# thomasantony/splat

Hardware: AMD Instinct MI355X
Metric: frames_per_sec (higher is better)
Workload: dtype f32

## Files before the change

### splat_amd/csrc/splat_api.hip

```cpp
#include <algorithm>
#include <cmath>
#include <cstdio>
#include <cstdlib>
#include <cstring>
#include <mutex>
#include <new>
#include <string>
#include <unordered_map>
#include <vector>

#include "splat_context.h"

using namespace splat;

static thread_local std::string g_create_error;
static std::mutex g_ledger_mu;
static std::unordered_map<void*, std::pair<splat_ctx*, size_t>> g_ledger;

namespace splat {
CommState** ctx_comm_slot(splat_ctx* c) { return &c->comm; }
hipStream_t ctx_stream(splat_ctx* c) { return c->stream; }
hipStream_t frame_stream(splat_ctx* c) { return (c->last_lane && c->comp2) ? c->comp2 : c->stream; }
int frame_tail(splat_ctx* c) {
    if (c->last_ring < 0 || !c->ring[c->last_ring].used) return SPLAT_OK;
// ... 491 lines not shown
        HIP_TRY(c, hipEventRecord(s.ev_ready, f.ss));
        HIP_TRY(c, hipStreamWaitEvent(cs, s.ev_ready, 0));
    }
    if (retained) launch_status_set(cs, f.d_st, c->ret_set.status);
    HIP_TRY(c, f.mark(5, cs));
    uint2* iters = nullptr;
    c->iters_valid = false;
    if (want_iters) {
        if (c->iters_alloc < m * 4u) {
            dfree(c->d_iters); c->iters_alloc = 0;
            HIP_TRY(c, dmalloc(c, &c->d_iters, sizeof(uint2) * (size_t)m * 4u));
            c->iters_alloc = m * 4u;
        }
        HIP_TRY(c, hipMemsetAsync(c->d_iters, 0, sizeof(uint2) * (size_t)m * 4u, cs));
        iters = c->d_iters;
        c->iters_valid = true;
    }
    CompositeArgs comp{};
    comp.s = cs; comp.knobs = &c->knobs; comp.n_tiles = m; comp.fc = c->fc; comp.recs = s.recs; comp.argb = d_argb; comp.status = f.d_st; comp.orig = c->orig;
    comp.fused_sort_max = retained ? 0u : c->fused_sort_max; comp.iters = iters; comp.keep_keys = want_iters || f.retain == SPLAT_RETAIN_WRITER;
    comp.pair_walk = pd.pair_walk != 0;
    comp.libm_exp = (c->cfg.mode & SPLAT_MODE_LIBM_EXP) != 0; comp.clear_first = c->clear_first;
    comp.lists = f.lists; comp.lists.near_m = pd.near_cap ? s.near_m : nullptr;
    comp.keys = f.keys; comp.keys.keys2 = pd.comp_sorts != 0 ? s.keys2 : nullptr;
    if (retained) {
        const bool near = c->ret_set.near_cap != 0u;
        comp.lists.near_m = near ? s.near_m : nullptr; comp.keys.keys2 = near ? s.keys2 : nullptr;
    }
    comp.hints = hint_table(c);
    if (c->knobs.dbg_stage_cache != 0u && f.retain == SPLAT_RETAIN_WRITER) {
        const size_t waves = (size_t)c->m_alloc * 4u;
        if (!c->stage_nv || !c->stage_mask) {
            dfree(c->stage_nv); dfree(c->stage_mask);
            HIP_TRY(c, dmalloc(c, &c->stage_nv, sizeof(unsigned int) * waves));
            HIP_TRY(c, dmalloc(c, &c->stage_mask, sizeof(unsigned long long) * 32u * waves));
        }
        HIP_TRY(c, hipMemsetAsync(c->stage_nv, 0, sizeof(unsigned int) * waves, cs));
        c->ret_set.frames = 0;
    }
    if (retained && c->knobs.dbg_stage_cache != 0u && c->stage_nv && c->stage_mask) {
        comp.stage_nv = c->stage_nv; comp.stage_mask = c->stage_mask;
        if (c->knobs.dbg_stage_cache == 2u && c->ret_set.frames >= 2u)
            HIP_TRY(c, hipMemsetAsync(c->stage_mask, 0, sizeof(unsigned long long) * 32u * (size_t)c->m_alloc * 4u, cs));
        c->ret_set.frames++;
    }
    comp.refine = c->fc.close_width == 0.0f ? pd.refine : 0u;
    launch_composite(comp);
    c->last_near = retained ? c->ret_set.near_cap != 0u : pd.near_cap != 0u;
    HIP_TRY(c, f.mark(6, cs));
    if (want_iters) HIP_TRY(c, hipMemcpyAsync(&c->h_status[f.r], f.d_st, sizeof(FrameStatus), hipMemcpyDeviceToHost, cs));
    HIP_TRY(c, hipEventRecord(f.ev->e[7], cs));
    return SPLAT_OK;
}

int decide_retention(splat_ctx* c, const splat_camera* cam, int* action) {
    splat_retain_input in;
    std::memset(&in, 0, sizeof in);
    static_assert(sizeof(splat_camera) + 2 * sizeof(int32_t) <= sizeof in.cam, "the camera and the slab fit the decision's words");
    std::memcpy(in.cam, cam, sizeof(splat_camera));
    const int32_t slab[2] = {c->slab0, c->slab1};
    std::memcpy(reinterpret_cast<unsigned char*>(in.cam) + sizeof(splat_camera), slab, sizeof slab);
    in.epoch = c->bin_epoch; in.still_frames = c->pol.still_frames;
    in.enabled = (c->retain_lists != 0 && c->knobs.dbg_ntiles == 0u) ? 1 : 0;
    in.overlap = c->overlap; in.one_pass = c->fc.bucket_cap ? 1 : 0;
    splat_retain_decision d;
    const int wr = c->ret_set.ring;
    for (int pass = 0; pass < 2; ++pass) {
        if (c->ret.writer == 1u && wr >= 0) {
            const volatile FrameStatus* hs = &c->h_status[wr];
            in.writer_arrived = hs->arrived; in.writer_overflow = hs->overflow; in.writer_redone = hs->redone;
        }
        if (splat_retain_decide(&c->ret, &in, &d) != 0) return fail(c, SPLAT_ERR_INVALID, "retention refused its input");
        if (pass == 0 && d.wait_for_writer != 0 && wr >= 0 && c->ring[wr].used) {
            HIP_TRY(c, hipEventSynchronize(c->ring[wr].e[7]));
// ... 411 lines not shown
    if (const char* e5 = std::getenv("SPLAT_BUCKETS")) { c->use_buckets = std::atoi(e5) != 0; c->env_pinned |= 1u << SPLAT_OPT_ONE_PASS_BINNING; }
    if (const char* e7 = std::getenv("SPLAT_CULL")) { c->cull_blocks = std::atoi(e7) != 0; c->env_pinned |= 1u << SPLAT_OPT_BLOCK_CULLING; }
    if (const char* e8 = std::getenv("SPLAT_DBG_TIGHT_GRIDS")) c->tight_grids = std::atoi(e8) != 0;
    option_from_env(c, SPLAT_OPT_PAIR_WALK, "SPLAT_PAIR_BLEND", -1, 1);
    if (const char* e6 = std::getenv("SPLAT_BUCKET_BYTES")) { c->bucket_bytes = std::strtoull(e6, nullptr, 10); c->env_pinned |= 1u << SPLAT_OPT_KEY_BUFFER_BYTES; }
    option_from_env(c, SPLAT_OPT_REGION_SPARE, "SPLAT_REGION_SPARE", 1, 1e9);
    if (const char* er = std::getenv("SPLAT_OVERFLOW_REDO")) { c->overflow_redo = std::min(2, std::max(0, std::atoi(er))); c->env_pinned |= 1u << SPLAT_OPT_OVERFLOW_REDO; }
    if (const char* en = std::getenv("SPLAT_NEAR_KEYS")) {
        const int v = std::atoi(en);
        c->near_cap = v <= 0 ? 0u : (unsigned int)std::min(2048, std::max(64, v));
        c->env_pinned |= 1u << SPLAT_OPT_NEAR_SELECT_KEYS;
    }
    option_from_env(c, SPLAT_OPT_HOST_ZERO_COPY, "SPLAT_HOST_ZERO_COPY", 0, 1);
    option_from_env(c, SPLAT_OPT_COUNT_FIRST, "SPLAT_COUNT_FIRST", 0, 2);
    if (const char* kg = std::getenv("SPLAT_KEYS_PER_GAUSSIAN")) {
        const int v = std::atoi(kg);
        c->keys_per_gaussian = v <= 0 ? 0u : (unsigned int)std::min(256, std::max(4, v));
        c->env_pinned |= 1u << SPLAT_OPT_KEYS_PER_GAUSSIAN;
    }
    option_from_env(c, SPLAT_OPT_LARGE_SPLAT_TILES, "SPLAT_LARGE_TILES", -1, 1048576);
    option_from_env(c, SPLAT_OPT_LARGE_LIST_MIN, "SPLAT_LARGE_LIST_MIN", -1, 1e9);
    option_from_env(c, SPLAT_OPT_START_REFINE, "SPLAT_START_REFINE", 0, 1);
    option_from_env(c, SPLAT_OPT_RETAIN_LISTS, "SPLAT_RETAIN", 0, 1);
    if (const char* lm = std::getenv("SPLAT_LAYOUT_MOTION")) c->layout_motion = std::atoi(lm) != 0 ? 1 : 0;
    if (const char* k1 = std::getenv("SPLAT_SORT_RADIX_MIN")) c->knobs.sort_radix_min = (unsigned int)std::max(0, std::atoi(k1));
    if (const char* k2 = std::getenv("SPLAT_SCAN_THREADS")) c->knobs.scan_threads = std::atoi(k2);
    if (const char* k3 = std::getenv("SPLAT_DBG_NTILES")) c->knobs.dbg_ntiles = (unsigned int)std::max(0, std::atoi(k3));
    if (const char* k8 = std::getenv("SPLAT_DBG_SELECT_STRIDE")) c->knobs.dbg_select_stride = (unsigned int)std::max(0, std::atoi(k8));
    if (const char* k10 = std::getenv("SPLAT_START_HINTS")) { c->start_hints = std::min(2, std::max(0, std::atoi(k10))); c->env_pinned |= 1u << SPLAT_OPT_START_HINTS; }
    if (const char* k7 = std::getenv("SPLAT_DBG_ONE_PASS_SELECT")) c->one_pass_select = std::atoi(k7) != 0;
    if (const char* k11 = std::getenv("SPLAT_DBG_KEYS2_ENTRIES")) c->knobs.dbg_keys2_entries = std::strtoull(k11, nullptr, 10);
    if (const char* k9 = std::getenv("SPLAT_DBG_HINT_RADIUS")) c->knobs.dbg_hint_radius = std::atoi(k9);
    if (const char* k12 = std::getenv("SPLAT_DBG_SELECT_BLIND")) c->knobs.dbg_select_blind = std::atoi(k12) != 0 ? 1u : 0u;
    if (const char* k13 = std::getenv("SPLAT_DBG_STAGE_CACHE")) c->knobs.dbg_stage_cache = (unsigned int)std::min(2, std::max(0, std::atoi(k13)));
    if (const char* k5 = std::getenv("SPLAT_DBG_STARTS")) c->knobs.dbg_starts = std::atoi(k5) != 0 ? 1u : 0u;
    if (const char* k4 = std::getenv("SPLAT_COMP_LDS_PAD")) c->knobs.comp_lds_pad = (unsigned int)std::max(0, std::atoi(k4));
    if (const char* k1p = std::getenv("SPLAT_K1_LDS_PAD")) c->knobs.k1_lds_pad = (unsigned int)std::min(48 * 1024, std::max(0, std::atoi(k1p)));
    auto bail = [&](const char* what, hipError_t err) {
        g_create_error = std::string(what) + ": " + hipGetErrorString(err);
        splat_destroy(c);
        return SPLAT_ERR_HIP;
    };
    if ((e = hipSetDevice(cfg->device)) != hipSuccess) return bail("hipSetDevice", e);
    if ((e = init_device_kernels()) != hipSuccess) return bail("hipFuncSetAttribute", e);
    if ((e = hipStreamCreateWithFlags(&c->stream, hipStreamNonBlocking)) != hipSuccess) return bail("hipStreamCreate", e);
    c->own_stream = true;
    {
        int lo = 0, hi = 0;
        (void)hipDeviceGetStreamPriorityRange(&lo, &hi);
        int prio = c->pipeline >= 6 ? (lo + hi) / 2 : hi;
        if (const char* ep = std::getenv("SPLAT_BIN_PRIO")) prio = std::atoi(ep) > 0 ? hi : (std::atoi(ep) < 0 ? lo : (lo + hi) / 2);
        if ((e = hipStreamCreateWithPriority(&c->bin_stream, hipStreamNonBlocking, prio)) != hipSuccess) return bail("hipStreamCreate", e);
        if ((e = hipStreamCreateWithPriority(&c->sort_stream, hipStreamNonBlocking, prio)) != hipSuccess) return bail("hipStreamCreate", e);
    }
    if (c->overlap >= 2 && c->pipeline) { if ((e = ensure_copy_stream(c)) != hipSuccess) return bail("hipStreamCreate", e); c->comp2 = c->copy_stream; }
    for (Slot& s : c->slots) {
        if ((e = dmalloc(c, &s.d_status, sizeof(FrameStatus))) != hipSuccess) return bail("hipMalloc(status)", e);
        if ((e = fill_now(s.d_status, 0, sizeof(FrameStatus))) != hipSuccess) return bail("fill_now(status)", e);
        if ((e = hipEventCreateWithFlags(&s.ev_ready, hipEventDisableTiming)) != hipSuccess) return bail("hipEventCreate", e);
        if ((e = hipEventCreateWithFlags(&s.ev_binned, hipEventDisableTiming)) != hipSuccess) return bail("hipEventCreate", e);
    }
    if ((e = dmalloc(c, &c->d_status_ring, sizeof(FrameStatus) * EV_RING)) != hipSuccess) return bail("hipMalloc(status ring)", e);
    if ((e = fill_now(c->d_status_ring, 0, sizeof(FrameStatus) * EV_RING)) != hipSuccess) return bail("fill_now(status ring)", e);
    if ((e = hipHostMalloc(&c->h_status, sizeof(FrameStatus) * EV_RING, hipHostMallocCoherent)) != hipSuccess) return bail("hipHostMalloc(status)", e);
    std::memset(c->h_status, 0, sizeof(FrameStatus) * EV_RING);
    for (auto& s : c->ring)
// ... 489 lines not shown
    if (n != c->n) return fail(c, SPLAT_ERR_INVALID, "record count mismatch");
    if (n == 0) return SPLAT_OK;
    int rc = splat_sync(c);
    if (rc != SPLAT_OK) return rc;
    if (c->last_slot < 0) return fail(c, SPLAT_ERR_INVALID, "no frame rendered yet");
    rc = ensure_two_pass_buffers(c, c->slots[c->last_slot]);
    if (rc != SPLAT_OK) return rc;
    const Slot& s = c->slots[c->last_slot];
    std::vector<Rec> r(n); std::vector<float> d(n); std::vector<ushort4> q(n);
    HIP_TRY(c, hipMemcpy(r.data(), s.recs, sizeof(Rec) * n, hipMemcpyDeviceToHost));
    {
        bump_epoch(c);
        FrameConst fc = c->fc;
        fc.bucket_cap = 0; fc.cull_blocks = 0;
        Slot& sl = c->slots[c->last_slot];
        HIP_TRY(c, hipMemsetAsync(sl.counts, 0, sizeof(unsigned int) * ((size_t)c->n_tiles + 1), c->stream));
        sl.layout_valid = false; sl.flip = 0;
        HIP_TRY(c, hipMemsetAsync(s.d_status, 0, sizeof(FrameStatus), c->stream));
        BinArgs k1{};
        k1.s = c->stream; k1.knobs = &c->knobs; k1.scene = {c->n, c->planes, c->orig, nullptr}; k1.fc = fc; k1.recs = s.recs; k1.depth = s.depth; k1.rect = s.rect;
        k1.vislist = s.vislist; k1.bin.cursors = s.counts; k1.status = s.d_status;
        launch_preprocess(k1);
        HIP_TRY(c, hipMemsetAsync(s.counts, 0, sizeof(unsigned int) * ((size_t)c->n_tiles + 1), c->stream));
        HIP_TRY(c, hipMemsetAsync(s.d_status, 0, sizeof(FrameStatus), c->stream));
        HIP_TRY(c, hipStreamSynchronize(c->stream));
    }
    HIP_TRY(c, hipMemcpy(d.data(), s.depth, sizeof(float) * n, hipMemcpyDeviceToHost));
    HIP_TRY(c, hipMemcpy(q.data(), s.rect, sizeof(ushort4) * n, hipMemcpyDeviceToHost));
    rc = ensure_h_orig(c);
    if (rc != SPLAT_OK) return rc;
    for (uint64_t j = 0; j < n; ++j) {
        const uint64_t i = c->h_orig[j];
        splat_record& o = out[i];
        o.cx = r[j].a.x; o.cy = r[j].a.y; o.hx = r[j].a.z; o.hy = r[j].a.w;
        o.conic_a = r[j].b.x; o.conic_b = c->fc.y_up ? r[j].b.y : -r[j].b.y; o.conic_c = r[j].b.z; o.opacity = r[j].b.w;
        o.r = r[j].c.x; o.g = r[j].c.y; o.b = r[j].c.z; o.depth = d[j];
        o.px0 = q[j].x; o.px1 = q[j].y; o.py0 = q[j].z; o.py1 = q[j].w;
    }
    return SPLAT_OK;
}

#if SPLAT_K1X == 30 || SPLAT_K1X == 31
int splat_debug_k1_stamps(splat_ctx* c, unsigned long long* out, unsigned long long n_words) {
    if (!c || c->last_slot < 0) return SPLAT_ERR_INVALID;
    (void)sync_all(c);
    return hipMemcpy(out, c->slots[c->last_slot].depth, n_words * 8, hipMemcpyDeviceToHost) == hipSuccess ? SPLAT_OK : SPLAT_ERR_HIP;
}
int splat_debug_k1_hwid(splat_ctx* c, unsigned long long* out, unsigned long long n_words) {
    if (!c || c->last_slot < 0) return SPLAT_ERR_INVALID;
    (void)sync_all(c);
    return hipMemcpy(out, c->slots[c->last_slot].rect, n_words * 8, hipMemcpyDeviceToHost) == hipSuccess ? SPLAT_OK : SPLAT_ERR_HIP;
}
#endif

int splat_debug_near_state(splat_ctx* c, unsigned int* lens, unsigned int* near_m, unsigned int* need_hint, unsigned int m) {
    if (!c || c->last_slot < 0 || m != c->n_tiles) return SPLAT_ERR_INVALID;
    (void)sync_all(c);
    const Slot& s = c->slots[c->last_slot];
    bool ok = hipMemcpy(lens, s.lens, sizeof(unsigned int) * m, hipMemcpyDeviceToHost) == hipSuccess;
    ok = ok && hipMemcpy(near_m, s.near_m, sizeof(unsigned int) * m, hipMemcpyDeviceToHost) == hipSuccess;
    ok = ok && hipMemcpy(need_hint, hint_table(c).needs(), sizeof(unsigned int) * HintTable::NEED_PLANES * m, hipMemcpyDeviceToHost) == hipSuccess;
    return ok ? SPLAT_OK : SPLAT_ERR_HIP;
}

int splat_debug_probe_failures(splat_ctx* c, uint64_t* n) {
    if (!c || !n || c->last_slot < 0) return SPLAT_ERR_INVALID;
// ... 57 lines not shown
```

### splat_amd/csrc/splat_context.h

```cpp
#ifndef SPLAT_CONTEXT_H
#define SPLAT_CONTEXT_H
#include <string>
#include <vector>

#include "splat_internal.h"
#include "../../include/splat_policy.h"
#include "../../include/splat_retain.h"

#define HIP_TRY(ctx, expr)                                                                             \
    do {                                                                                               \
        hipError_t _e = (expr);                                                                        \
        if (_e != hipSuccess) {                                                                        \
            (ctx)->err = std::string(#expr) + ": " + hipGetErrorString(_e);                            \
            return SPLAT_ERR_HIP;                                                                      \
        }                                                                                              \
    } while (0)

namespace splat {
constexpr int N_EV = 9;
constexpr int N_TIMES = 6;
constexpr int EV_RING = 32;
static_assert(EV_RING == SPLAT_POLICY_RING, "the frame policy sees the whole status ring");
constexpr int N_SLOTS = 4;

// ... 82 lines not shown
    unsigned int* upd_bad = nullptr;
    unsigned char* upd_dirty = nullptr;
    float ply_ms[3] = {0.0f, 0.0f, 0.0f};
    float upload_sort_ms = 0.0f;
    splat::Slot slots[splat::N_SLOTS];
    unsigned int m_alloc = 0;
    uint64_t cap = 0;
    uint64_t cap2 = 0;
    uint64_t keys2_want = 0;
    bool use_buckets = true;
    bool bucket_failed = false;
    uint64_t bucket_bytes = 128ull << 30;
    uint64_t layout_want = 0;
    unsigned int layout_m = 0;
    bool last_one_pass = false;
    unsigned int* zero_layout = nullptr;
    uint64_t dev_bytes = 0, dev_bytes_peak = 0;
    splat::LaunchKnobs knobs;
    float region_spare = 4.0f;
    uint64_t frame_idx = 0;
    uint64_t bin_idx = 0;
    int retain_lists = 1;
    uint64_t bin_epoch = 0;
    splat_retain_state ret{};
    uint64_t frames_retained = 0;
    struct RetainSet {
        int slot = -1, ring = -1;
        unsigned int near_cap = 0;
        splat::FrameStatus status{};
        unsigned int frames = 0;
    } ret_set;
    unsigned int* stage_nv = nullptr;
    unsigned long long* stage_mask = nullptr;
    int last_slot = -1;
    bool last_lists_in_memory = false;
    splat::FrameStatus* h_status = nullptr;
    splat::FrameStatus* d_status_ring = nullptr;
    bool clear_first = false;
    uint32_t* d_img = nullptr;
    size_t img_cap = 0;
    static constexpr int S_IMGS = 4;
    uint32_t* s_img[S_IMGS] = {};
    size_t s_cap = 0;
    hipStream_t copy_stream = nullptr;
    hipEvent_t s_rendered[S_IMGS] = {}, s_copied[S_IMGS] = {};
    const uint32_t* s_dst[S_IMGS] = {};
    bool s_used[S_IMGS] = {};
    uint64_t s_idx = 0;
    int s_ring[S_IMGS] = {-1, -1, -1, -1};
    splat_camera s_cam[S_IMGS] = {};
    int slab0 = 0, slab1 = -1;
    splat::EvSet ring[splat::EV_RING];
    int ring_next = 0;
    int last_ring = -1;
    double acc_ms[splat::N_TIMES] = {0, 0, 0, 0, 0, 0};
    uint64_t acc_frames = 0;
    splat::FrameConst fc{};
    unsigned int n_tiles = 0;
    uint64_t overflow_want = 0;
    bool bucket_overflow = false;
    bool sort_hint = false, sort_grid_miss = false;
    unsigned int hint_ge8192 = 0, hint_ge2048 = 0, hint_ge16384 = 0;
    int pair_mode = -1;
    uint64_t hint_pairs = 0; unsigned int hint_maxlen = 0; unsigned int hint_large = 0, hint_window = 0;
    unsigned int grid_big = 0, grid_mid = 0, grid_long = 0;
    splat::FrameStatus last{};
// ... 48 lines not shown
```

### splat_amd/csrc/splat_internal.h

```cpp
#ifndef SPLAT_INTERNAL_H
#define SPLAT_INTERNAL_H
#include <hip/hip_runtime.h>
#include <stdint.h>

#include "../../include/splat_hip.h"

#ifndef SPLAT_K1X
#define SPLAT_K1X 0
#endif
#ifndef SPLAT_EXP_STAGE2
#define SPLAT_EXP_STAGE2 0
#endif
#ifndef SPLAT_EXP_K1DUMMY
#define SPLAT_EXP_K1DUMMY 0
#endif
#ifndef SPLAT_EXP_SKIPFULL
#define SPLAT_EXP_SKIPFULL 0
#endif
#ifndef SPLAT_EXP_SORT2
#define SPLAT_EXP_SORT2 0
#endif
#ifndef SPLAT_EXP_K1DROP
#define SPLAT_EXP_K1DROP 0
#endif

namespace splat {

constexpr int TILE = SPLAT_TILE;
constexpr int SCENE_PLANES = 16;
constexpr int LIVE_PLANES = 10;


struct FrameConst {
    float view[16];
    float proj[16];
    float w, h;
    float htanx, htany, focal;
    float cam[3];
    float lowpass;
    int sh_dim;
    int y_up, sample_half, zclip;
    float zmin, zmax;
    int W, H;
    int tiles_x;
// ... 26 lines not shown
    unsigned long long n_sort_fallback;
    unsigned int n_near_tiles;
    unsigned int n_near_fallback;
    unsigned int n_large;
    unsigned int n_window;
    unsigned int n_ge8192, n_ge2048;
    unsigned int n_ge16384;
    unsigned int redone;
    unsigned int n_long_keys;
    unsigned int arrived;
    unsigned int n_probe_fail;
    unsigned int pad_;
    unsigned long long n_blocks_culled;
    unsigned long long layout_total;
};

struct Rec {
    float4 a;
    float4 b;
    float4 c;
};

struct LaunchKnobs {
    unsigned int sort_radix_min = 128;
    int scan_threads = 0;
    unsigned int dbg_ntiles = 0;
    unsigned int comp_lds_pad = 0;
    unsigned int k1_lds_pad = 0;
    unsigned int dbg_select_stride = 0;
    unsigned long long dbg_keys2_entries = 0;
    int dbg_hint_radius = -1;
    unsigned int dbg_select_blind = 0;
    unsigned int dbg_starts = 0;
    unsigned int dbg_stage_cache = 1;
};

struct HintTable {
    unsigned int* base;
    size_t stride;

    static constexpr unsigned int NEED_PLANE = 0u, NEED_PLANES = 4u;
    static constexpr unsigned int DEPTH_PLANE = NEED_PLANE + NEED_PLANES, DEPTH_PLANES = 1u;
    static constexpr unsigned int START_PLANE = DEPTH_PLANE + DEPTH_PLANES, START_PLANES = 4u;
    static constexpr unsigned int REFINE_PLANE = START_PLANE + START_PLANES, REFINE_PLANES = 4u;
    static constexpr unsigned int HINT_WORDS = 13u;
    static_assert(DEPTH_PLANE == 4u && START_PLANE == 5u && REFINE_PLANE == 9u && REFINE_PLANE + REFINE_PLANES == HINT_WORDS,
                  "the four parts tile the table exactly");

    unsigned int* plane(unsigned int k) const { return base ? base + k * stride : nullptr; }
    unsigned int* needs() const { return plane(NEED_PLANE); }
    unsigned int* select_depth() const { return plane(DEPTH_PLANE); }
    unsigned int* starts() const { return plane(START_PLANE); }
    unsigned int* refinement() const { return plane(REFINE_PLANE); }
    size_t words() const { return HINT_WORDS * stride; }
    size_t bytes() const { return sizeof(unsigned int) * words(); }
};

void launch_pack_scene(hipStream_t s, uint64_t n, const float* pos4, const float* cov3d, const float* opacity,
                       const float* sh, const unsigned int* perm, float4* planes);
void launch_cov3d(hipStream_t s, uint64_t n, const float* scales3, const float* rot4, float* cov3d);
size_t scene_order_small_bytes(uint64_t n);
void launch_scene_order(hipStream_t s, uint64_t n, const float* pos4, uint32_t* pingpong, void* small, unsigned int* orig,
                        hipEvent_t sort_begin = nullptr, hipEvent_t sort_end = nullptr);
void launch_block_bounds(hipStream_t s, uint64_t n, const float* pos4, const float* cov3d, const unsigned int* orig, BlockBounds* bounds);

void launch_ply_decode(hipStream_t s, const splat_ply_layout& lay, const void* d_rows, float* pos4, float* scales3,
// ... 106 lines not shown
struct SortArgs {
    hipStream_t s; const LaunchKnobs* knobs; unsigned int n_tiles; SortGrids grids; TileLists lists; KeyBuffers keys; FrameStatus* status;
    const unsigned int* orig;
    unsigned int fused_sort_max;
};
void launch_sort(const SortArgs& a);

struct SelectArgs {
    hipStream_t s; const LaunchKnobs* knobs; unsigned int n_tiles; TileLists lists; KeyBuffers keys; FrameStatus* status;
    const unsigned int* orig;
    unsigned int near_cap;
    const unsigned int* need_hint;
    unsigned int* near_thr;
    unsigned int tiles_x, tile_rows;
    unsigned int grid;
    bool at_rest;
    int hint_radius;
};
void launch_select(const SelectArgs& a);

struct CompositeArgs {
    hipStream_t s; const LaunchKnobs* knobs; unsigned int n_tiles; FrameConst fc;
    TileLists lists;
    KeyBuffers keys;
    const Rec* recs; uint32_t* argb; FrameStatus* status; const unsigned int* orig;
    unsigned int fused_sort_max;
    uint2* iters;
    bool keep_keys;
    bool pair_walk;
    bool libm_exp;
    bool clear_first;
    HintTable hints;
    unsigned int refine;
    unsigned int* stage_nv;
    unsigned long long* stage_mask;
};
void launch_composite(const CompositeArgs& a);
void launch_status_set(hipStream_t s, FrameStatus* status, const FrameStatus& v);
hipError_t init_device_kernels();

struct CommState;
CommState** ctx_comm_slot(splat_ctx* c);
hipStream_t ctx_stream(splat_ctx* c);
hipStream_t frame_stream(splat_ctx* c);
int ctx_device(const splat_ctx* c);
int frame_tail(splat_ctx* c);
int ctx_quiesce(splat_ctx* c);
int ctx_fail(splat_ctx* c, int code, const char* msg);
void comm_release(CommState* s);

}
#endif
```

### splat_amd/csrc/splat_kernels.hip

```cpp
#include <algorithm>
#include <cstddef>
#include <cstdlib>
#include <type_traits>

#include "splat_internal.h"
#include "splat_device_math.h"

namespace splat {
static constexpr unsigned long long KERNELS_EXP2F_TAB[32] = {
    0x3ff0000000000000ull, 0x3fefd9b0d3158574ull, 0x3fefb5586cf9890full, 0x3fef9301d0125b51ull, 0x3fef72b83c7d517bull,
    0x3fef54873168b9aaull, 0x3fef387a6e756238ull, 0x3fef1e9df51fdee1ull, 0x3fef06fe0a31b715ull, 0x3feef1a7373aa9cbull,
    0x3feedea64c123422ull, 0x3feece086061892dull, 0x3feebfdad5362a27ull, 0x3feeb42b569d4f82ull, 0x3feeab07dd485429ull,
    0x3feea47eb03a5585ull, 0x3feea09e667f3bcdull, 0x3fee9f75e8ec5f74ull, 0x3feea11473eb0187ull, 0x3feea589994cce13ull,
    0x3feeace5422aa0dbull, 0x3feeb737b0cdc5e5ull, 0x3feec49182a3f090ull, 0x3feed503b23e255dull, 0x3feee89f995ad3adull,
    0x3feeff76f2fb5e47ull, 0x3fef199bdd85529cull, 0x3fef3720dcef9069ull, 0x3fef5818dcfba487ull, 0x3fef7c97337b9b5full,
    0x3fefa4afa2a490daull, 0x3fefd0765b6e4540ull};
constexpr bool exp2f_tab_is_the_headers() {
    for (int i = 0; i < 32; ++i) if (KERNELS_EXP2F_TAB[i] != EXP2F_TAB_HOST[i]) return false;
    return true;
}
static_assert(exp2f_tab_is_the_headers(), "splat_kernels.hip's copy of EXP2F_TAB differs from splat_device_math.h's");
}


// ... 2245 lines not shown
    unsigned long long* h = keys2 + off2[tile];
    merge(g, r1, g + r1, r2 - r1, h);
    merge(g + r2, r3 - r2, g + r3, n - r3, h + r2);
    __syncthreads();
    merge(h, r2, h + r2, n - r2, g);
}

__device__ __forceinline__ unsigned long long uniform_u64(unsigned long long v) {
    return ((unsigned long long)(unsigned int)__builtin_amdgcn_readfirstlane((int)(v >> 32)) << 32) |
           (unsigned long long)(unsigned int)__builtin_amdgcn_readfirstlane((int)(unsigned int)v);
}

struct WaveLds { float4 a[64]; float4 b[64]; float4 c[64]; };

#ifndef SPLAT_REFINE_MIN_STEP
#define SPLAT_REFINE_MIN_STEP 8
#endif
#ifndef SPLAT_COMP_WAVES
#define SPLAT_COMP_WAVES 1
#endif
struct CompArgs {
    FrameConst fc;
    const unsigned int* offsets; const unsigned int* order; const unsigned int* lens;
    unsigned long long* keys; const Rec* recs; uint32_t* argb; FrameStatus* status;
    unsigned int fused_sort_max, radix_min;
    uint2* iters;
    unsigned int keep_keys, clear_first;
    const unsigned int* orig;
    unsigned long long* keys2; const unsigned int* near_m;
    unsigned int* need_hint; unsigned int* start_hint; const unsigned int* off2;
    unsigned int* probe_hint;
    unsigned int refine;
    unsigned int* stage_nv; unsigned long long* stage_mask;
};
typedef const __attribute__((address_space(4))) CompArgs* KernArgs;
template <bool PAIR, bool LIBM, bool KEEP>
static __device__ void repair_tile(KernArgs ka, unsigned int smem_lds, unsigned int exptab_lds, unsigned int item, bool again);

template <bool PAIR, bool LIBM, int LONGM, bool KEEP = false>
__device__ __forceinline__ void composite_tile(unsigned char* smem, const unsigned long long* exptab, const unsigned int item, const FrameConst& fc,
                                               const unsigned int* __restrict__ offsets, const unsigned int* __restrict__ order,
                                               const unsigned int* __restrict__ lens, unsigned long long* __restrict__ keys,
                                               const Rec* __restrict__ recs, uint32_t* __restrict__ argb,
                                               FrameStatus* __restrict__ status, unsigned int fused_sort_max,
                                               unsigned int radix_min, uint2* __restrict__ iters, unsigned int keep_keys,
                                               const unsigned int* __restrict__ orig, const unsigned int clear_first,
                                               unsigned long long* __restrict__ keys2, const unsigned int* __restrict__ near_m,
                                               unsigned int* __restrict__ need_hint, unsigned int* __restrict__ start_hint,
                                               const unsigned int* __restrict__ off2, KernArgs ka ,
                                               const bool walk_this_wave = true, const bool second_walk = false ) {
    auto late = [&]() -> KernArgs {
        unsigned long long p = (unsigned long long)(size_t)ka;
        asm volatile("" : "+s"(p));
        return (KernArgs)(size_t)p;
    };
    static_assert(sizeof(WaveLds) * 4 <= sort_lds_bytes<256, 2048>(), "staging fits the sort workspace");
    WaveLds* slds = reinterpret_cast<WaveLds*>(smem);
    const unsigned int tile = (unsigned int)__builtin_amdgcn_readfirstlane((int)order[item]);
    const unsigned int tid = threadIdx.x;
    const unsigned int beg = __builtin_amdgcn_readfirstlane(offsets[tile]);
    const unsigned int end = beg + __builtin_amdgcn_readfirstlane(lens[tile]);
    if (beg == end) {
        if (clear_first) {
            const KernArgs k = late();
            const int tiles_x = k->fc.tiles_x, W = k->fc.W, H = k->fc.H, r0 = k->fc.row_px0, r1 = k->fc.row_px1;
            const int txx0 = (int)(tile % (unsigned int)tiles_x), tyy0 = (int)(tile / (unsigned int)tiles_x) + k->fc.tile_row0;
// ... 279 lines not shown
                B2 = blend_channel(B2, ia, ab);
            }
        };
        blend_one(alpha0, (f2){q4.x, q4.y}, q5.x);
        blend_one(alpha1, (f2){q4.z, q4.w}, q5.z);
    };
    auto run = [&](auto BRt, unsigned int start) -> unsigned int {
        constexpr bool BR = decltype(BRt)::value;
        Rec r;
        unsigned int kb = start < end ? (end - 1u - start) >> 6 : 0u;
        unsigned int bsN = start, cntN = start < end ? (end - (kb << 6)) - start : 0u;
        if (cntN) fetch(bsN, cntN, r);
        while (cntN) {
            const unsigned int bs = bsN, cnt = cntN;
            const bool reuse = kb < nA;
            const unsigned int abase = (end - lb >= ((kb + 1u) << 6)) ? end - ((kb + 1u) << 6) : lb;
            const bool keep = KEEP && keeping && !reuse && kb < 32u && bs == abase;
            const unsigned int k = stage(r, cnt, bs, true, false, PAIR, reuse ? (int)kb : -1, bs - abase, keep ? (int)kb : -1);
            bsN = bs + cnt; cntN = min(64u, end - bsN); kb -= cntN ? 1u : 0u;
            if (cntN) fetch(bsN, cntN, r);
            if constexpr (PAIR) {
                const float4* P4 = reinterpret_cast<const float4*>(&L);
                for (unsigned int j = 0; j < (k + 1u) / 2u; ++j)
                    shade_pair(BRt, P4[6 * j], P4[6 * j + 1], P4[6 * j + 2], P4[6 * j + 3], P4[6 * j + 4], P4[6 * j + 5]);
            } else {
                for (unsigned int j = 0; j < k; ++j) shade(BRt, L.a[j], L.b[j], L.c[j]);
            }
            itB += k;
            if (BR && __builtin_amdgcn_ballot_w64(inside & ((R2 - R > cw) | (G2 - G > cw) | (B2 - B > cw))) == 0ull) return bsN;
        }
        return end;
    };
    unsigned int start = ws;
    while (!need_far) {
        if (start <= lb) {
            if (has_far) { need_far = true; break; }
            R = (float)((old >> 16) & 0xffu); G = (float)((old >> 8) & 0xffu); B = (float)(old & 0xffu);
            run(std::false_type{}, lb);
            break;
        }
        R = G = B = 0.0f; R2 = G2 = B2 = 255.0f;
        const unsigned int pos = run(std::true_type{}, start);
        const bool open = __builtin_amdgcn_ballot_w64(inside & ((R2 - R > cw) | (G2 - G > cw) | (B2 - B > cw))) != 0ull;
        if (!open) {
            R = truncf((R + R2) * 0.5f); G = truncf((G + G2) * 0.5f); B = truncf((B + B2) * 0.5f);
            if (pos < end) run(std::false_type{}, pos);
            break;
        }
        if (probe != 0u && !(probe >> 31)) {
            probe |= 0x80000000u;
            const KernArgs kr = late();
            const unsigned int g = (unsigned int)__builtin_amdgcn_readfirstlane((int)kr->start_hint[tile * 4u + wave]);
            if (lane == 0) atomicAdd(&kr->status->n_probe_fail, 1u);
            if (g > end - start && g < end - lb) { start = end - g; continue; }
        }
        if (lane == 0) atomicAdd(&late()->status->n_fallback, 1ull);
        const unsigned int depth = end - start;
        start = (start - lb > depth) ? start - depth : lb;
    }
    const float A = (alast < 0.0f) ? (float)(old >> 24) : truncf(alast * 255.0f);
    const KernArgs kl = late();
    uint2* const iters_l = kl->iters;
    if (iters_l != nullptr && lane == 0) {
        const unsigned int kk = kl->keep_keys;
        uint2 v = (kk & 2u) ? make_uint2(end - beg, end - max(start, beg)) : make_uint2(itA, itB);
        if (second_walk && !(kk & 2u)) { const uint2 o = iters_l[item * 4u + wave]; v.x += o.x; v.y += o.y; }
        iters_l[item * 4u + wave] = v;
    }
    if constexpr (LONGM != 0) {
        unsigned int* const need_l = kl->need_hint;
        if (need_l != nullptr && end - beg > 2048u && lane == 0u) need_l[tile * 4u + wave] = need_far ? 0xffffffffu : end - max(start, lb);
    }
    unsigned int* const start_l = kl->start_hint;
    if (start_l != nullptr && early && !need_far && (scanned || start != ws) && lane == 0u) {
        unsigned int used = max(end - max(start, lb), 1u);
        if (!has_far && used > (end - beg) - ((end - beg) >> 2)) used = end - beg;
        start_l[tile * 4u + wave] = used;
    }
    if (probe != 0u && lane == 0u) {
        const bool failed = (probe >> 31) != 0u;
        const unsigned int half = (probe & 0xffffu) >> 1;
        const unsigned int step = failed ? (half >= (unsigned int)SPLAT_REFINE_MIN_STEP ? half : 0u) : probe;
        if (!failed) start_l[tile * 4u + wave] = end - ws;
        kl->probe_hint[tile * 4u + wave] = (kl->refine & 0xffff0000u) | step;
    }
    if (KEEP && keeping && !need_far && max(start, lb) < end) {
        const unsigned int s = max(start, lb), kf = (end - 1u - s) >> 6;
        const unsigned int ab = (end - lb >= ((kf + 1u) << 6)) ? end - ((kf + 1u) << 6) : lb;
        const unsigned int nv_new = min(kf + (s == ab ? 1u : 0u), 32u);
        unsigned int* const nv_l = kl->stage_nv;
        const unsigned int nv_old = (unsigned int)__builtin_amdgcn_readfirstlane((int)nv_l[tile * 4u + wave]);
        if (nv_new > nv_old) {
            __builtin_amdgcn_fence(__ATOMIC_RELEASE, "wavefront");
            __builtin_amdgcn_wave_barrier();
            if (lane >= nv_old && lane < nv_new) kl->stage_mask[(size_t)(tile * 4u + wave) * 32u + lane] = wmask[lane];
            if (lane == 0u) nv_l[tile * 4u + wave] = nv_new;
            __builtin_amdgcn_fence(__ATOMIC_ACQUIRE, "wavefront");
            __builtin_amdgcn_wave_barrier();
        }
    }
    if (need_far) return true;
    if (inside)
        kl->argb[(size_t)py * kl->fc.W + px] = ((uint32_t)A << 24) | ((uint32_t)R << 16) | ((uint32_t)G << 8) | (uint32_t)B;
    return false;
    };
    if constexpr (LONGM != 2) {
        (void)walk_list();
    } else {
        const bool again = walk_list();
        if (has_far && __syncthreads_or(again ? 1 : 0) != 0) {
            if (tid == 0u) atomicAdd(&late()->status->n_near_fallback, 1u);
            repair_tile<PAIR, LIBM, KEEP>(ka, (unsigned int)(size_t)(__attribute__((address_space(3))) unsigned char*)smem,
                                    (unsigned int)(size_t)(__attribute__((address_space(3))) const unsigned long long*)exptab, item, again);
        }
    }
}

template <bool PAIR, bool LIBM, bool KEEP>
static __device__ __attribute__((noinline)) void repair_tile(KernArgs ka, unsigned int smem_lds, unsigned int exptab_lds, unsigned int item, bool again) {
    const unsigned long long kp = uniform_u64((unsigned long long)(size_t)ka);
    const KernArgs k = (KernArgs)(size_t)kp;
    unsigned char* const smem = (unsigned char*)(__attribute__((address_space(3))) unsigned char*)(size_t)__builtin_amdgcn_readfirstlane((int)smem_lds);
    const unsigned long long* const exptab = (const unsigned long long*)(__attribute__((address_space(3))) const unsigned long long*)(size_t)__builtin_amdgcn_readfirstlane((int)exptab_lds);
    const unsigned int it = (unsigned int)__builtin_amdgcn_readfirstlane((int)item);
    FrameConst fc;
    {
        const __attribute__((address_space(4))) unsigned int* src = (const __attribute__((address_space(4))) unsigned int*)&k->fc;
        unsigned int* dst = reinterpret_cast<unsigned int*>(&fc);
#pragma unroll
        for (unsigned int q = 0; q < sizeof(FrameConst) / 4u; ++q) dst[q] = src[q];
    }
    composite_tile<PAIR, LIBM, 1>(smem, exptab, it, fc, k->offsets, k->order, k->lens, k->keys, k->recs, k->argb, k->status, k->fused_sort_max, k->radix_min,
                                  k->iters, k->keep_keys, k->orig, k->clear_first, k->keys2, nullptr, k->need_hint, k->start_hint, k->off2, k, again, true);
    if (threadIdx.x == 0u) {
        const unsigned int tile = k->order[it];
        const_cast<unsigned int*>(k->near_m)[tile] = k->lens[tile];
        unsigned int* const nv_l = KEEP ? k->stage_nv : nullptr;
        if (nv_l != nullptr) { nv_l[tile * 4u + 0u] = 0u; nv_l[tile * 4u + 1u] = 0u; nv_l[tile * 4u + 2u] = 0u; nv_l[tile * 4u + 3u] = 0u; }
    }
}

__global__ __launch_bounds__(256) void select_near_kernel(const unsigned int* __restrict__ offsets, const unsigned int* __restrict__ order,
                                                          const unsigned int* __restrict__ lens, unsigned long long* __restrict__ keys,
                                                          unsigned long long* __restrict__ keys2, FrameStatus* __restrict__ status,
                                                          const unsigned int* __restrict__ orig, unsigned int radix_min, unsigned int near_cap,
                                                          const unsigned int* __restrict__ need_hint, unsigned int* __restrict__ near_m,
                                                          unsigned int tiles_x, unsigned int tile_rows, unsigned int* __restrict__ near_thr,
                                                          unsigned int n_slots, unsigned int at_rest, const unsigned int* __restrict__ off2,
                                                          int hint_radius, unsigned int blind) {
    __shared__ __attribute__((aligned(16))) unsigned char smem[sort_lds_bytes<256, 2048>()];
    if (status->overflow) return;
  for (unsigned int slot = blockIdx.x; slot < n_slots; slot += gridDim.x) {
    const unsigned int tile = (unsigned int)__builtin_amdgcn_readfirstlane((int)order[slot]);
    const unsigned int n = (unsigned int)__builtin_amdgcn_readfirstlane((int)lens[tile]);
    if (n < 2048u) return;
    if (n == 2048u) continue;
    const unsigned int beg = (unsigned int)__builtin_amdgcn_readfirstlane((int)offsets[tile]);
    unsigned long long* const k2 = keys2 + (unsigned int)__builtin_amdgcn_readfirstlane((int)off2[tile]);
    unsigned int want = near_cap, deepest, thr = 0u;
    {
        unsigned int* const word = reinterpret_cast<unsigned int*>(smem);
        if (threadIdx.x < 64u) {
            const uint4 h4 = reinterpret_cast<const uint4*>(need_hint)[tile];
            unsigned int d0 = max(max(h4.x, h4.y), max(h4.z, h4.w));
            if (hint_radius > 0) {
                const int D = 2 * hint_radius + 1;
                unsigned int nb = 0u;
                for (int idx = (int)threadIdx.x; idx < D * D; idx += 64) {
                    const int tx = (int)(tile % tiles_x) + idx % D - hint_radius, ty = (int)(tile / tiles_x) + idx / D - hint_radius;
                    if (tx >= 0 && ty >= 0 && tx < (int)tiles_x && ty < (int)tile_rows) {
                        const uint4 q = reinterpret_cast<const uint4*>(need_hint)[(unsigned int)ty * tiles_x + (unsigned int)tx];
// ... 231 lines not shown
                               status, orig, off2);
    }
    if (grid_mid)
    hipLaunchKernelGGL((sort_tiles_kernel<512, 8192>), dim3(grid_mid), dim3(512), (sort_lds_bytes<512, 8192>()), s, offsets, order,
                       lens, keys, keys2, status, 2048u, radix_min, 0, 0u, 1u, orig, off2);
    if (fused_sort_max < 2048u)
        hipLaunchKernelGGL((sort_tiles_kernel<256, 2048>), dim3(n_tiles), dim3(256), (sort_lds_bytes<256, 2048>()), s, offsets, order,
                           lens, keys, keys2, status, fused_sort_max, radix_min, 0, 0u, 1u, orig, off2);
}
void launch_select(const SelectArgs& a) {
    const unsigned int n_tiles = a.n_tiles;
    if (!n_tiles) return;
    const unsigned int* off2 = a.lists.off2;
    if (!off2) off2 = a.lists.offsets;
    int hint_radius = a.hint_radius;
    unsigned int grid = a.grid;
    if (a.knobs->dbg_hint_radius >= 0) hint_radius = a.knobs->dbg_hint_radius;
    if (a.knobs->dbg_select_stride) grid = (n_tiles + a.knobs->dbg_select_stride - 1u) / a.knobs->dbg_select_stride;
    if (!grid) grid = (n_tiles + 7u) / 8u;
    hipLaunchKernelGGL(select_near_kernel, dim3(std::min(grid, n_tiles)), dim3(256), 0, a.s, a.lists.offsets, a.lists.order, a.lists.lens, a.keys.keys, a.keys.keys2, a.status, a.orig, a.knobs->sort_radix_min,
                       std::min(std::max(a.near_cap, 64u), 2048u), a.need_hint, a.lists.near_m, a.tiles_x, a.tile_rows, a.near_thr, n_tiles, a.at_rest ? 1u : 0u, off2, std::min(std::max(hint_radius, 0), 7), a.knobs->dbg_select_blind);
}
void launch_composite(const CompositeArgs& c) {
    unsigned int n_tiles = c.n_tiles;
    if (!n_tiles) return;
    const unsigned int* off2 = c.lists.off2;
    if (!off2) off2 = c.lists.offsets;
    if (c.knobs->dbg_ntiles) n_tiles = std::min(n_tiles, c.knobs->dbg_ntiles);
    const unsigned int pad = c.knobs->comp_lds_pad;
    unsigned long long* keys2 = c.keys.keys2;
    const unsigned int* near_m = c.lists.near_m;
    unsigned int *need_hint = c.hints.needs(), *start_hint = c.hints.starts(), *probe_hint = c.hints.refinement();
    const bool near = near_m != nullptr && keys2 != nullptr && need_hint != nullptr;
    const unsigned int flags = (c.keep_keys ? 1u : 0u) | (c.knobs->dbg_starts ? 2u : 0u);
    CompArgs a;
    a.fc = c.fc; a.offsets = c.lists.offsets; a.order = c.lists.order; a.lens = c.lists.lens; a.keys = c.keys.keys; a.recs = c.recs; a.argb = c.argb; a.status = c.status;
    a.fused_sort_max = c.fused_sort_max; a.radix_min = c.knobs->sort_radix_min; a.iters = c.iters; a.keep_keys = flags; a.clear_first = c.clear_first ? 1u : 0u;
    a.orig = c.orig; a.keys2 = keys2; a.near_m = near_m; a.need_hint = near ? need_hint : nullptr; a.start_hint = start_hint; a.off2 = off2;
    a.probe_hint = probe_hint; a.refine = (probe_hint != nullptr && start_hint != nullptr) ? c.refine : 0u;
    const bool keep_verdicts = c.stage_nv != nullptr && c.stage_mask != nullptr && (near || keys2 == nullptr);
    a.stage_nv = keep_verdicts ? c.stage_nv : nullptr; a.stage_mask = keep_verdicts ? c.stage_mask : nullptr;
    auto go = [&](auto kern) { hipLaunchKernelGGL(kern, dim3(n_tiles), dim3(256), pad, c.s, a); };
    if (keep_verdicts && near) {
        if (c.libm_exp) go(composite_retained_kernel<false, true, 2>);
        else if (c.pair_walk) go(composite_retained_kernel<true, false, 2>);
        else go(composite_retained_kernel<false, false, 2>);
    } else if (keep_verdicts) {
        if (c.libm_exp) go(composite_retained_kernel<false, true, 0>);
        else if (c.pair_walk) go(composite_retained_kernel<true, false, 0>);
        else go(composite_retained_kernel<false, false, 0>);
    } else if (near) {
        if (c.libm_exp) go(composite_exact_kernel<false, true, 2>);
        else if (c.pair_walk) go(composite_exact_kernel<true, false, 2>);
        else go(composite_exact_kernel<false, false, 2>);
    } else if (keys2 != nullptr) {
        if (c.libm_exp) go(composite_exact_kernel<false, true, 1>);
        else if (c.pair_walk) go(composite_exact_kernel<true, false, 1>);
        else go(composite_exact_kernel<false, false, 1>);
    } else {
        if (c.libm_exp) go(composite_exact_kernel<false, true, 0>);
        else if (c.pair_walk) go(composite_exact_kernel<true, false, 0>);
        else go(composite_exact_kernel<false, false, 0>);
    }
}

}
```

Measured before the change: 5156.

## Cache proven composite start per wave to skip bracket pass on retained frames

New measurement: 5591, median of 6. 8.4% higher.

```diff
diff --git a/splat_amd/csrc/splat_api.hip b/splat_amd/csrc/splat_api.hip
--- a/splat_amd/csrc/splat_api.hip
+++ b/splat_amd/csrc/splat_api.hip
@@ -547,14 +547,15 @@
         const size_t waves = (size_t)c->m_alloc * 4u;
         if (!c->stage_nv || !c->stage_mask) {
             dfree(c->stage_nv); dfree(c->stage_mask);
-            HIP_TRY(c, dmalloc(c, &c->stage_nv, sizeof(unsigned int) * waves));
+            HIP_TRY(c, dmalloc(c, &c->stage_nv, sizeof(unsigned int) * 2u * waves));
             HIP_TRY(c, dmalloc(c, &c->stage_mask, sizeof(unsigned long long) * 32u * waves));
         }
-        HIP_TRY(c, hipMemsetAsync(c->stage_nv, 0, sizeof(unsigned int) * waves, cs));
+        HIP_TRY(c, hipMemsetAsync(c->stage_nv, 0, sizeof(unsigned int) * 2u * waves, cs));
         c->ret_set.frames = 0;
     }
     if (retained && c->knobs.dbg_stage_cache != 0u && c->stage_nv && c->stage_mask) {
         comp.stage_nv = c->stage_nv; comp.stage_mask = c->stage_mask;
+        if (c->knobs.dbg_proven_starts != 0u && c->fc.close_width == 0.0f) comp.proven_start = c->proven_start();
         if (c->knobs.dbg_stage_cache == 2u && c->ret_set.frames >= 2u)
             HIP_TRY(c, hipMemsetAsync(c->stage_mask, 0, sizeof(unsigned long long) * 32u * (size_t)c->m_alloc * 4u, cs));
         c->ret_set.frames++;
@@ -1032,6 +1033,8 @@
     if (const char* k11 = std::getenv("SPLAT_DBG_KEYS2_ENTRIES")) c->knobs.dbg_keys2_entries = std::strtoull(k11, nullptr, 10);
     if (const char* k9 = std::getenv("SPLAT_DBG_HINT_RADIUS")) c->knobs.dbg_hint_radius = std::atoi(k9);
     if (const char* k12 = std::getenv("SPLAT_DBG_SELECT_BLIND")) c->knobs.dbg_select_blind = std::atoi(k12) != 0 ? 1u : 0u;
+    if (const char* k15 = std::getenv("SPLAT_DBG_PROVEN_STARTS")) c->knobs.dbg_proven_starts = (unsigned int)std::min(2, std::max(0, std::atoi(k15)));
+    if (const char* k14 = std::getenv("SPLAT_DBG_BRACKET_COUNT")) c->knobs.dbg_bracket_count = std::atoi(k14) != 0 ? 1u : 0u;
     if (const char* k13 = std::getenv("SPLAT_DBG_STAGE_CACHE")) c->knobs.dbg_stage_cache = (unsigned int)std::min(2, std::max(0, std::atoi(k13)));
     if (const char* k5 = std::getenv("SPLAT_DBG_STARTS")) c->knobs.dbg_starts = std::atoi(k5) != 0 ? 1u : 0u;
     if (const char* k4 = std::getenv("SPLAT_COMP_LDS_PAD")) c->knobs.comp_lds_pad = (unsigned int)std::max(0, std::atoi(k4));
@@ -1587,6 +1590,8 @@
     for (uint64_t j = 0; j < n; ++j) {
         const uint64_t i = c->h_orig[j];
         splat_record& o = out[i];
+        const bool on_target = q[j].x <= q[j].y && q[j].z <= q[j].w;
+        if (!(on_target && std::max((int)q[j].z, c->fc.row_px0) <= std::min((int)q[j].w, c->fc.row_px1 - 1))) r[j] = Rec{};
         o.cx = r[j].a.x; o.cy = r[j].a.y; o.hx = r[j].a.z; o.hy = r[j].a.w;
         o.conic_a = r[j].b.x; o.conic_b = c->fc.y_up ? r[j].b.y : -r[j].b.y; o.conic_c = r[j].b.z; o.opacity = r[j].b.w;
         o.r = r[j].c.x; o.g = r[j].c.y; o.b = r[j].c.z; o.depth = d[j];
diff --git a/splat_amd/csrc/splat_context.h b/splat_amd/csrc/splat_context.h
--- a/splat_amd/csrc/splat_context.h
+++ b/splat_amd/csrc/splat_context.h
@@ -138,6 +138,7 @@
     } ret_set;
     unsigned int* stage_nv = nullptr;
     unsigned long long* stage_mask = nullptr;
+    unsigned int* proven_start() const { return stage_nv ? stage_nv + (size_t)m_alloc * 4u : nullptr; }
     int last_slot = -1;
     bool last_lists_in_memory = false;
     splat::FrameStatus* h_status = nullptr;
diff --git a/splat_amd/csrc/splat_internal.h b/splat_amd/csrc/splat_internal.h
--- a/splat_amd/csrc/splat_internal.h
+++ b/splat_amd/csrc/splat_internal.h
@@ -10,6 +10,9 @@
 #endif
 #ifndef SPLAT_EXP_STAGE2
 #define SPLAT_EXP_STAGE2 0
+#endif
+#ifndef SPLAT_EXP_NO_BRACKET
+#define SPLAT_EXP_NO_BRACKET 0
 #endif
 #ifndef SPLAT_EXP_K1DUMMY
 #define SPLAT_EXP_K1DUMMY 0
@@ -102,6 +105,8 @@
     int dbg_hint_radius = -1;
     unsigned int dbg_select_blind = 0;
     unsigned int dbg_starts = 0;
+    unsigned int dbg_bracket_count = 0;
+    unsigned int dbg_proven_starts = 1;
     unsigned int dbg_stage_cache = 1;
 };
 
@@ -274,6 +279,7 @@
     bool clear_first;
     HintTable hints;
     unsigned int refine;
+    unsigned int* proven_start;
     unsigned int* stage_nv;
     unsigned long long* stage_mask;
 };
diff --git a/splat_amd/csrc/splat_kernels.hip b/splat_amd/csrc/splat_kernels.hip
--- a/splat_amd/csrc/splat_kernels.hip
+++ b/splat_amd/csrc/splat_kernels.hip
@@ -2301,6 +2301,7 @@
     unsigned int* probe_hint;
     unsigned int refine;
     unsigned int* stage_nv; unsigned long long* stage_mask;
+    unsigned int* proven_start;
 };
 typedef const __attribute__((address_space(4))) CompArgs* KernArgs;
 template <bool PAIR, bool LIBM, bool KEEP>
@@ -2646,6 +2647,13 @@
         return end;
     };
     unsigned int start = ws;
+    if constexpr (KEEP) {
+        if (cw == 0.0f && hinted && probe == 0u && !second_walk && start > lb) {
+            const KernArgs kp = late();
+            const unsigned int* const pv_l = kp->proven_start;
+            if (pv_l != nullptr && (unsigned int)__builtin_amdgcn_readfirstlane((int)pv_l[tile * 4u + wave]) == end - start) probe = 0x20000000u;
+        }
+    }
     while (!need_far) {
         if (start <= lb) {
             if (has_far) { need_far = true; break; }
@@ -2653,12 +2661,24 @@
             run(std::false_type{}, lb);
             break;
         }
+#if SPLAT_EXP_NO_BRACKET
+        if (KEEP && cw == 0.0f && hinted && probe == 0u && !second_walk) { R = G = B = 0.0f; run(std::false_type{}, start); break; }
+#endif
         R = G = B = 0.0f; R2 = G2 = B2 = 255.0f;
-        const unsigned int pos = run(std::true_type{}, start);
+        unsigned int pos = start;
+        if (KEEP && probe == 0x20000000u) {
+            if (late()->keep_keys & 8u) R = G = B = 255.0f;
+            R2 = R; G2 = G; B2 = B;
+        } else {
+            if constexpr (KEEP) { if (late()->keep_keys & 4u) itA -= itB; }
+            pos = run(std::true_type{}, start);
+            if constexpr (KEEP) { if (late()->keep_keys & 4u) itA += itB; }
+        }
         const bool open = __builtin_amdgcn_ballot_w64(inside & ((R2 - R > cw) | (G2 - G > cw) | (B2 - B > cw))) != 0ull;
         if (!open) {
             R = truncf((R + R2) * 0.5f); G = truncf((G + G2) * 0.5f); B = truncf((B + B2) * 0.5f);
             if (pos < end) run(std::false_type{}, pos);
+            if constexpr (KEEP) probe = (probe & 0x20000000u) ? 0u : (probe | 0x40000000u);
             break;
         }
         if (probe != 0u && !(probe >> 31)) {
@@ -2691,12 +2711,18 @@
         if (!has_far && used > (end - beg) - ((end - beg) >> 2)) used = end - beg;
         start_l[tile * 4u + wave] = used;
     }
+    const unsigned int closed_here = KEEP ? probe & 0x40000000u : 0u;
+    if constexpr (KEEP) probe &= 0x8000ffffu;
     if (probe != 0u && lane == 0u) {
         const bool failed = (probe >> 31) != 0u;
         const unsigned int half = (probe & 0xffffu) >> 1;
         const unsigned int step = failed ? (half >= (unsigned int)SPLAT_REFINE_MIN_STEP ? half : 0u) : probe;
         if (!failed) start_l[tile * 4u + wave] = end - ws;
         kl->probe_hint[tile * 4u + wave] = (kl->refine & 0xffff0000u) | step;
+    }
+    if constexpr (KEEP) {
+        unsigned int* const pv_l = kl->proven_start;
+        if (closed_here != 0u && !need_far && pv_l != nullptr && lane == 0u) pv_l[tile * 4u + wave] = end - start;
     }
     if (KEEP && keeping && !need_far && max(start, lb) < end) {
         const unsigned int s = max(start, lb), kf = (end - 1u - s) >> 6;
@@ -2751,6 +2777,8 @@
         const_cast<unsigned int*>(k->near_m)[tile] = k->lens[tile];
         unsigned int* const nv_l = KEEP ? k->stage_nv : nullptr;
         if (nv_l != nullptr) { nv_l[tile * 4u + 0u] = 0u; nv_l[tile * 4u + 1u] = 0u; nv_l[tile * 4u + 2u] = 0u; nv_l[tile * 4u + 3u] = 0u; }
+        unsigned int* const pv_l = KEEP ? k->proven_start : nullptr;
+        if (pv_l != nullptr) { pv_l[tile * 4u + 0u] = 0u; pv_l[tile * 4u + 1u] = 0u; pv_l[tile * 4u + 2u] = 0u; pv_l[tile * 4u + 3u] = 0u; }
     }
 }
 
@@ -3048,7 +3076,8 @@
     const unsigned int* near_m = c.lists.near_m;
     unsigned int *need_hint = c.hints.needs(), *start_hint = c.hints.starts(), *probe_hint = c.hints.refinement();
     const bool near = near_m != nullptr && keys2 != nullptr && need_hint != nullptr;
-    const unsigned int flags = (c.keep_keys ? 1u : 0u) | (c.knobs->dbg_starts ? 2u : 0u);
+    const unsigned int flags = (c.keep_keys ? 1u : 0u) | (c.knobs->dbg_starts ? 2u : 0u) | (c.knobs->dbg_bracket_count ? 4u : 0u) |
+                               (c.knobs->dbg_proven_starts == 2u ? 8u : 0u);
     CompArgs a;
     a.fc = c.fc; a.offsets = c.lists.offsets; a.order = c.lists.order; a.lens = c.lists.lens; a.keys = c.keys.keys; a.recs = c.recs; a.argb = c.argb; a.status = c.status;
     a.fused_sort_max = c.fused_sort_max; a.radix_min = c.knobs->sort_radix_min; a.iters = c.iters; a.keep_keys = flags; a.clear_first = c.clear_first ? 1u : 0u;
@@ -3056,6 +3085,7 @@
     a.probe_hint = probe_hint; a.refine = (probe_hint != nullptr && start_hint != nullptr) ? c.refine : 0u;
     const bool keep_verdicts = c.stage_nv != nullptr && c.stage_mask != nullptr && (near || keys2 == nullptr);
     a.stage_nv = keep_verdicts ? c.stage_nv : nullptr; a.stage_mask = keep_verdicts ? c.stage_mask : nullptr;
+    a.proven_start = (keep_verdicts && c.fc.close_width == 0.0f) ? c.proven_start : nullptr;
     auto go = [&](auto kern) { hipLaunchKernelGGL(kern, dim3(n_tiles), dim3(256), pad, c.s, a); };
     if (keep_verdicts && near) {
         if (c.libm_exp) go(composite_retained_kernel<false, true, 2>);
```
